# HansBambel/SmaAt-UNet

Hardware: NVIDIA H100
Metric: SmaAt-UNet fwd frames/sec @ B=32 12×288×288; depthwise % HBM roofline (higher is better)
Workload: dtype f32

## Files before the change

smaat_unet_b200/csrc/dsconv_fused.cu:

```cuda
#include <stdlib.h>

#include "tc_common.cuh"

namespace smaat {

struct DsParams {
  const float* dw_w;
  const float* dw_b;
  const float* scale;
  const float* shift;
  float* y;
  int64_t y_bstride;
  double* stats;
  const float* oc_w;
  const float* oc_b;
  float* oc_y;
  int C0, C1, H, W, Cout, relu, K;
  int tiles_x, tiles_y, npass, total_tiles, nchunks;
};

template <int N_TILE, int KPL, int PW, bool X3, bool A_SMEM>
struct DsCfg {
  static constexpr int PH = TC_BM / PW;
  static constexpr int BW = PW + 8, BH = PH + 2;
  static constexpr int CC = TC_BK / KPL;
  static constexpr int IN_BYTES = CC * BH * BW * 4;
  static constexpr int A_BYTES = TC_BM * TC_BK * 4;
  static constexpr int B_BYTES = N_TILE * TC_BK * 4;
  static constexpr int AST_BYTES = (X3 && A_SMEM ? 2 : 1) * A_BYTES;
  static constexpr int BST_BYTES = (X3 ? 2 : 1) * B_BYTES;
  static constexpr int OFF_ALO = A_BYTES;
  static constexpr int OFF_BLO = B_BYTES;
  static constexpr int NG = N_TILE > 64 ? 1 : 2;
  static constexpr int AS = X3 ? (A_SMEM ? (N_TILE > 64 ? 2 : 3) : 2 + NG) : 4;
  static constexpr int BS = X3 ? (A_SMEM && N_TILE > 64 ? 2 : 3) : 4;
  static constexpr int AFF_N = 512;
  static constexpr int BAR_BYTES = 512;
  static constexpr int IS_FIT = (224 * 1024 - 1024 - BAR_BYTES - 3 * AFF_N * 4 - AS * AST_BYTES - BS * BST_BYTES) / IN_BYTES;
  static constexpr int IS = IS_FIT > 8 ? 8 : IS_FIT;
  static constexpr int OFF_A = ((IS * IN_BYTES + 1023) / 1024) * 1024;
  static constexpr int OFF_BR = OFF_A + AS * AST_BYTES;
  static constexpr int OFF_BAR = OFF_BR + BS * BST_BYTES;
  static_assert((IS * NG + IS + 2 * AS + 2 * BS) * 8 <= BAR_BYTES, "barrier block");
  static constexpr int TOTAL = OFF_BAR + BAR_BYTES + 3 * AFF_N * 4 + 1024;
  static constexpr uint32_t B_TX = BST_BYTES;
  static constexpr int PROD_WARP = 12;
  static constexpr int THREADS = 384 + 128 * NG;
  static constexpr int REGS_LAUNCH = (65536 / THREADS) / 8 * 8;
  static constexpr int REGS_TMA = 24;
  static constexpr int REGS_PROD = N_TILE > 64 ? 104 : REGS_LAUNCH;
  static constexpr int REGS_MMA = ((THREADS / 128 * REGS_LAUNCH - REGS_TMA - NG * REGS_PROD) / 2) / 8 * 8;
  static constexpr int REGS_SUM = REGS_TMA + 2 * REGS_MMA + NG * REGS_PROD;
  static_assert(REGS_SUM <= THREADS / 128 * REGS_LAUNCH && REGS_MMA >= REGS_LAUNCH, "register budget");
  static constexpr int KS = (X3 && N_TILE == 64) ? 2 : TC_BK / 8;
  static_assert(IS >= 2, "input ring");
  static_assert(NG <= AS, "phase-parity barriers");
  static_assert(IN_BYTES % 128 == 0, "TMA destination alignment");
  static_assert(TOTAL <= 227 * 1024, "shared memory budget");
};

template <int N_TILE, int KPL, int PW, bool X3, bool A_SMEM>
__global__ void __launch_bounds__(DsCfg<N_TILE, KPL, PW, X3, A_SMEM>::THREADS, 1)
    dsconv_fused_kernel(const __grid_constant__ CUtensorMap map_in0, const __grid_constant__ CUtensorMap map_in1,
                        const __grid_constant__ CUtensorMap map_w, const __grid_constant__ CUtensorMap map_wlo,
                        const DsParams p) {
  using L = DsCfg<N_TILE, KPL, PW, X3, A_SMEM>;
  constexpr int PH = L::PH, BW = L::BW, BH = L::BH, CC = L::CC, IS = L::IS, AS = L::AS, BS = L::BS;
  extern __shared__ __align__(1024) unsigned char smem_dyn[];
  unsigned char* smem = smem_dyn + ((1024u - (smem_u32(smem_dyn) & 1023u)) & 1023u);
  unsigned char* a_base = smem + L::OFF_A;
  unsigned char* b_base = smem + L::OFF_BR;
  uint64_t* bars = reinterpret_cast<uint64_t*>(smem + L::OFF_BAR);
  uint64_t* in_full = bars;
  uint64_t* in_empty = in_full + IS * L::NG;
  uint64_t* a_full = in_empty + IS;
  uint64_t* a_empty = a_full + AS;
  uint64_t* b_full = a_empty + AS;
  uint64_t* b_empty = b_full + BS;
  float* aff = reinterpret_cast<float*>(smem + L::OFF_BAR + L::BAR_BYTES);

  const int warp = __shfl_sync(0xffffffffu, (int)(threadIdx.x >> 5), 0);
  const int lane = threadIdx.x & 31;
  const int nch = p.nchunks;
  const int tiles_per_img = p.tiles_x * p.tiles_y * p.npass;
  auto decode = [&](int tile, int& b, int& ty, int& tx, int& np) {
    b = tile / tiles_per_img;
    int t2 = tile - b * tiles_per_img;
    np = t2 % p.npass;
    t2 /= p.npass;
    ty = t2 / p.tiles_x;
    tx = t2 - ty * p.tiles_x;
  };

  if (warp == 0 && lane == 0) {
    tma_prefetch_desc(&map_in0);
    tma_prefetch_desc(&map_in1);
    tma_prefetch_desc(&map_w);
    if (X3) tma_prefetch_desc(&map_wlo);
    for (int s = 0; s < IS; ++s) {
      for (int g = 0; g < L::NG; ++g) mbar_init(&in_full[s * L::NG + g], 1);
      mbar_init(&in_empty[s], 128);
    }
    for (int s = 0; s < AS; ++s) {
      mbar_init(&a_full[s], 128);
      mbar_init(&a_empty[s], 8);
    }
    for (int s = 0; s < BS; ++s) {
      mbar_init(&b_full[s], 1);
      mbar_init(&b_empty[s], 8);
    }
    fence_barrier_init();
  }
  for (int c = threadIdx.x; c < L::AFF_N; c += blockDim.x) {
    aff[c] = (c < p.Cout && p.scale) ? __ldg(p.scale + c) : 1.f;
    aff[L::AFF_N + c] = (c < p.Cout && p.shift) ? __ldg(p.shift + c) : 0.f;
    aff[2 * L::AFF_N + c] = (c < p.Cout && p.oc_w) ? __ldg(p.oc_w + c) : 0.f;
  }
  __syncthreads();

  if (warp < 4) {
    regs_dealloc<L::REGS_TMA>();
    if (warp == 0 && lane == 0) {
      uint32_t gc = 0;
      for (int tile = blockIdx.x; tile < p.total_tiles; tile += gridDim.x) {
        int b, ty, tx, np;
        decode(tile, b, ty, tx, np);
        const int x0 = tx * PW, y0 = ty * PH;
        for (int i = 0; i < nch; ++i, ++gc) {
          const int s = gc % IS;
          mbar_wait(&in_empty[s], ((gc / IS) & 1u) ^ 1u);
          uint64_t* full = &in_full[s * L::NG + (int)(gc % (uint32_t)L::NG)];
          mbar_arrive_expect_tx(full, L::IN_BYTES);
          const int cb = i * CC;
          const CUtensorMap* m = (cb < p.C0) ? &map_in0 : &map_in1;
          const int cc = (cb < p.C0) ? cb : cb - p.C0;
          asm volatile(
              "cp.async.bulk.tensor.4d.shared::cluster.global.mbarrier::complete_tx::bytes [%0], [%1, {%3, %4, %5, %6}], [%2];" ::
                  "r"(smem_u32(smem + s * L::IN_BYTES)),
              "l"(reinterpret_cast<uint64_t>(m)), "r"(smem_u32(full)), "r"(x0 - 4), "r"(y0 - 1), "r"(cc), "r"(b)
              : "memory");
        }
      }
    }
    if (warp == 1 && lane == 0) {
      uint32_t gc = 0;
      for (int tile = blockIdx.x; tile < p.total_tiles; tile += gridDim.x) {
        int b, ty, tx, np;
        decode(tile, b, ty, tx, np);
        for (int i = 0; i < nch; ++i, ++gc) {
          const int sb = gc % BS;
          mbar_wait(&b_empty[sb], ((gc / BS) & 1u) ^ 1u);
          mbar_arrive_expect_tx(&b_full[sb], L::B_TX);
          tma_load_2d(b_base + sb * L::BST_BYTES, &map_w, &b_full[sb], i * TC_BK, np * N_TILE);
          if (X3) tma_load_2d(b_base + sb * L::BST_BYTES + L::OFF_BLO, &map_wlo, &b_full[sb], i * TC_BK, np * N_TILE);
        }
      }
    }
    return;
  }

  if (warp < L::PROD_WARP) {
    regs_alloc<L::REGS_MMA>();
    const int wg = (warp >> 2) - 1, wq = warp & 3;
    const int g = lane >> 2, t = lane & 3;
    const int m0 = A_SMEM ? 64 * wg + 16 * wq + g : tc_row_pixel(wg, wq, 0, g);
    const int m1 = A_SMEM ? m0 + 8 : tc_row_pixel(wg, wq, 1, g);
    const float act_lo = p.relu ? 0.f : -INFINITY;
    const int64_t P = (int64_t)p.H * p.W;
    uint32_t gc = 0;
    for (int tile = blockIdx.x; tile < p.total_tiles; tile += gridDim.x) {
      int b, ty, tx, np;
      decode(tile, b, ty, tx, np);
      float acc[N_TILE / 2];
#pragma unroll
      for (int i = 0; i < N_TILE / 2; ++i) acc[i] = 0.f;
      auto release = [&](uint32_t c) {
        __syncwarp();
        if (lane == 0) {
          mbar_arrive(&a_empty[c % AS]);
          mbar_arrive(&b_empty[c % BS]);
        }
      };
      auto wait_stages = [&](const unsigned char*& ast, uint64_t& bd, uint64_t& bl) {
        const int sa = gc % AS, sb = gc % BS;
        mbar_wait(&a_full[sa], (gc / AS) & 1u);
        mbar_wait(&b_full[sb], (gc / BS) & 1u);
        ast = a_base + sa * L::AST_BYTES;
        bd = make_kmajor_desc(smem_u32(b_base + sb * L::BST_BYTES));
        bl = make_kmajor_desc(smem_u32(b_base + sb * L::BST_BYTES + L::OFF_BLO));
      };
      if (A_SMEM) {
        for (int i = 0; i < nch; ++i, ++gc) {
          const unsigned char* ast;
          uint64_t bd0, bl0;
          wait_stages(ast, bd0, bl0);
          const uint32_t a_addr = smem_u32(ast) + (uint32_t)(wg * 64 * 128);
          const uint64_t ad0 = make_kmajor_desc(a_addr), al0 = make_kmajor_desc(a_addr + L::OFF_ALO);
          wgmma_fence();
#pragma unroll
          for (int kk = 0; kk < TC_BK / 8; ++kk) {
            Wgmma<N_TILE>::ss(acc, ad0 + (uint64_t)(2 * kk), bd0 + (uint64_t)(2 * kk), 1u);
            if (X3) {
              Wgmma<N_TILE>::ss(acc, al0 + (uint64_t)(2 * kk), bd0 + (uint64_t)(2 * kk), 1u);
              Wgmma<N_TILE>::ss(acc, ad0 + (uint64_t)(2 * kk), bl0 + (uint64_t)(2 * kk), 1u);
            }
          }
          wgmma_commit();
          wgmma_wait<1>();
          if (i > 0) release(gc - 1);
        }
        wgmma_wait0();
      } else {
        constexpr int KS = L::KS, GPC = (TC_BK / 8) / KS;
        const unsigned char* ast = nullptr;
        uint64_t bd0 = 0, bl0 = 0;
        auto group = [&](AFrags<X3, KS>& cur, AFrags<X3, KS>& prev, int q) {
          const int part = q % GPC;
          if (part == 0) wait_stages(ast, bd0, bl0);
          load_a_frags<X3, KS>(ast, part * KS, t, m0, m1, cur);
          mma_a_frags<N_TILE, X3, KS>(acc, cur, bd0, bl0, part * KS);
          wgmma_wait<1>();
          wgmma_keep(prev);
          if (part == 0 && q > 0) release(gc - 1);
          if (part == GPC - 1) ++gc;
        };
        AFrags<X3, KS> fa, fb;
        const int ngrp = nch * GPC;
        int q = 0;
        for (; q + 1 < ngrp; q += 2) {
          group(fa, fb, q);
          group(fb, fa, q + 1);
        }
        if (q < ngrp) group(fa, fb, q);
        wgmma_wait0();
        wgmma_keep(fa);
        wgmma_keep(fb);
      }
      wgmma_keep(acc);
      release(gc - 1);

      const int n0 = np * N_TILE;
      const int gy0 = ty * PH + m0 / PW, gx0 = tx * PW + m0 % PW;
      const int gy1 = ty * PH + m1 / PW, gx1 = tx * PW + m1 % PW;
      const bool v0 = gy0 < p.H && gx0 < p.W, v1 = gy1 < p.H && gx1 < p.W;
      const int64_t o0 = (int64_t)gy0 * p.W + gx0, o1 = (int64_t)gy1 * p.W + gx1;
      if (p.stats) {
        const double npix = (double)((__popc(__ballot_sync(0xffffffffu, v0)) + __popc(__ballot_sync(0xffffffffu, v1))) / 4);
#pragma unroll
        for (int j = 0; j < N_TILE / 8; ++j) {
#pragma unroll
          for (int e = 0; e < 2; ++e) {
            const float a = v0 ? acc[4 * j + e] : 0.f, bb = v1 ? acc[4 * j + 2 + e] : 0.f;
            const float s1 = frag_colsum(a + bb), s2 = frag_colsum(fmaf(a, a, bb * bb));
            const int c = 8 * j + 2 * t + e;
            if (lane < 4 && c < p.Cout) {
              const double sc = (double)aff[c], sh = (double)aff[L::AFF_N + c];
              atomicAdd(p.stats + c, sc * (double)s1 + npix * sh);
              atomicAdd(p.stats + p.Cout + c, sc * sc * (double)s2 + 2.0 * sc * sh * (double)s1 + npix * sh * sh);
            }
          }
        }
      }
      if (p.oc_y) {
        float d0 = 0.f, d1 = 0.f;
#pragma unroll
        for (int j = 0; j < N_TILE / 8; ++j) {
#pragma unroll
          for (int e = 0; e < 2; ++e) {
            const int c = 8 * j + 2 * t + e;
            const float sc = aff[c], sh = aff[L::AFF_N + c], w = aff[2 * L::AFF_N + c];
            d0 = fmaf(fmaxf(fmaf(acc[4 * j + e], sc, sh), act_lo), w, d0);
            d1 = fmaf(fmaxf(fmaf(acc[4 * j + 2 + e], sc, sh), act_lo), w, d1);
          }
        }
        d0 += __shfl_xor_sync(0xffffffffu, d0, 1);
        d0 += __shfl_xor_sync(0xffffffffu, d0, 2);
        d1 += __shfl_xor_sync(0xffffffffu, d1, 1);
        d1 += __shfl_xor_sync(0xffffffffu, d1, 2);
        const float ob = p.oc_b ? __ldg(p.oc_b) : 0.f;
        if (t == 0) {
          if (v0) p.oc_y[(int64_t)b * P + o0] = d0 + ob;
          if (v1) p.oc_y[(int64_t)b * P + o1] = d1 + ob;
        }
      } else {
        float* yb = p.y + (int64_t)b * p.y_bstride;
#pragma unroll
        for (int j = 0; j < N_TILE / 8; ++j) {
#pragma unroll
          for (int e = 0; e < 2; ++e) {
            const int c = n0 + 8 * j + 2 * t + e;
            if (c < p.Cout) {
              const float sc = aff[c], sh = aff[L::AFF_N + c];
              float* yc = yb + (int64_t)c * P;
              if (v0) yc[o0] = fmaxf(fmaf(acc[4 * j + e], sc, sh), act_lo);
              if (v1) yc[o1] = fmaxf(fmaf(acc[4 * j + 2 + e], sc, sh), act_lo);
            }
          }
        }
      }
    }
    return;
  }

  {
    if (L::REGS_PROD < L::REGS_LAUNCH) regs_dealloc<L::REGS_PROD>();
    const int g = (warp - L::PROD_WARP) >> 2;
    const int t = threadIdx.x - 32 * L::PROD_WARP - 128 * g;
    const int Cin = p.C0 + p.C1;
    uint32_t gc = 0, iph = 0;
    for (int tile = blockIdx.x; tile < p.total_tiles; tile += gridDim.x) {
      for (int i = 0; i < nch; ++i, ++gc) {
        if ((int)(gc % (uint32_t)L::NG) != g) continue;
        const int s = gc % IS;
        float wr[KPL][9], br[KPL];
        auto task_channel = [&](int task) { return (PW == 32) ? (task >> 3) : (((task >> 4) << 1) | ((task >> 2) & 1)); };
        auto load_weights = [&](int task) {
          const int gch = i * CC + task_channel(task);
          const bool chv = gch < Cin;
#pragma unroll
          for (int kk = 0; kk < KPL; ++kk) {
            const int gk = gch * KPL + kk;
#pragma unroll
            for (int w9 = 0; w9 < 9; ++w9) wr[kk][w9] = chv ? __ldg(p.dw_w + (int64_t)gk * 9 + w9) : 0.f;
            br[kk] = (chv && p.dw_b) ? __ldg(p.dw_b + gk) : 0.f;
          }
        };
        load_weights(t);
        mbar_wait(&in_full[s * L::NG + g], (iph >> s) & 1u);
        iph ^= 1u << s;
        const int sa = gc % AS;
        mbar_wait(&a_empty[sa], ((gc / AS) & 1u) ^ 1u);
        unsigned char* my_op = a_base + sa * L::AST_BYTES;
        const float* in_stage = reinterpret_cast<const float*>(smem + s * L::IN_BYTES);
#pragma unroll 1
        for (int task = t; task < CC * 8; task += 128) {
          int ci, qc, rg;
          if (PW == 32) {
            ci = task >> 3; qc = task & 7; rg = 0;
          } else {
            qc = task & 3; ci = ((task >> 4) << 1) | ((task >> 2) & 1); rg = (task >> 3) & 1;
          }
          constexpr int NQ = PW / 4;
          const int c0 = qc << 2, r0 = rg << 2;
          if (task != t) load_weights(task);
          const float* trow = in_stage + (ci * BH + r0) * BW + c0 + 3;
          float win[3][6];
          const bool lb = (qc == 0), rb = (qc == NQ - 1);
          const int edge = lb ? 0 : 5;
          auto load_row = [&](float* wl, int r) {
            const float4 a = *reinterpret_cast<const float4*>(trow + r * BW + 1);
            float left = __shfl_up_sync(0xffffffffu, a.w, 1), right = __shfl_down_sync(0xffffffffu, a.x, 1);
            if (lb | rb) {
              const float e = trow[r * BW + edge];
              if (lb) left = e; else right = e;
            }
            wl[0] = left; wl[1] = a.x; wl[2] = a.y; wl[3] = a.z; wl[4] = a.w; wl[5] = right;
          };
#pragma unroll
          for (int r = 0; r < 2; ++r) load_row(win[r], r);
#pragma unroll
          for (int rr = 0; rr < 4; ++rr) {
            load_row(win[(rr + 2) % 3], rr + 2);
            const float* w0 = win[rr % 3];
            const float* w1 = win[(rr + 1) % 3];
            const float* w2 = win[(rr + 2) % 3];
            const int m = (r0 + rr) * PW + c0;
#pragma unroll
            for (int kk = 0; kk < KPL; ++kk) {
              float o4[4];
#pragma unroll
              for (int j = 0; j < 4; ++j) {
                float a = br[kk];
                a = fmaf(wr[kk][0], w0[j], a); a = fmaf(wr[kk][1], w0[j + 1], a); a = fmaf(wr[kk][2], w0[j + 2], a);
                a = fmaf(wr[kk][3], w1[j], a); a = fmaf(wr[kk][4], w1[j + 1], a); a = fmaf(wr[kk][5], w1[j + 2], a);
                a = fmaf(wr[kk][6], w2[j], a); a = fmaf(wr[kk][7], w2[j + 1], a); a = fmaf(wr[kk][8], w2[j + 2], a);
                o4[j] = a;
              }
              if (A_SMEM) {
                const int kr = ci * KPL + kk;
#pragma unroll
                for (int j = 0; j < 4; ++j) {
                  const uint32_t off = kmajor_offset(m + j, kr);
                  const float h = X3 ? tf32_hi(o4[j]) : o4[j];
                  *reinterpret_cast<float*>(my_op + off) = h;
                  if (X3) *reinterpret_cast<float*>(my_op + L::OFF_ALO + off) = o4[j] - h;
                }
                continue;
              }
              *reinterpret_cast<float4*>(my_op + a_tile_offset(ci * KPL + kk, m)) = make_float4(o4[0], o4[1], o4[2], o4[3]);
            }
          }
        }
        if (A_SMEM) fence_proxy_async_smem();
        mbar_arrive(&a_full[sa]);
        mbar_arrive(&in_empty[s]);
      }
    }
  }
}

template <int N_TILE, int KPL, int PW, bool X3, bool A_SMEM>
static int launch_ds(const CUtensorMap& m0, const CUtensorMap& m1, const CUtensorMap& mw, const CUtensorMap& mwl, DsParams p,
                     int B, cudaStream_t st) {
  using L = DsCfg<N_TILE, KPL, PW, X3, A_SMEM>;
  auto kern = dsconv_fused_kernel<N_TILE, KPL, PW, X3, A_SMEM>;
  static std::atomic<uint64_t> attr_mask{0};
  if (first_use_on_device(attr_mask)) {
    cudaError_t e = cudaFuncSetAttribute(kern, cudaFuncAttributeMaxDynamicSharedMemorySize, L::TOTAL);
    if (e != cudaSuccess) return fail(SMAAT_E_CUDA, "dsconv: smem attribute (%d B): %s", L::TOTAL, cudaGetErrorString(e));
    int r = check_reg_budget((const void*)kern, L::THREADS, L::REGS_SUM, "dsconv");
    if (r) return r;
  }
  p.tiles_x = ceil_div(p.W, PW);
  p.tiles_y = ceil_div(p.H, L::PH);
  p.npass = ceil_div(p.Cout, N_TILE);
  const int64_t total = (int64_t)B * p.tiles_x * p.tiles_y * p.npass;
  SMAAT_REQUIRE(total < (1ll << 31), "dsconv: too many tiles");
  p.total_tiles = (int)total;
  p.nchunks = ceil_div(p.C0 + p.C1, L::CC);
  const int grid = p.total_tiles < num_sms() ? p.total_tiles : num_sms();
  kern<<<grid, L::THREADS, L::TOTAL, st>>>(m0, m1, mw, mwl, p);
  SMAAT_LAUNCH_CHECK("smaat_dsconv_fwd");
  return SMAAT_OK;
}

static int pick_pw(int H, int W) {
  double best = 1e9;
  int pw = 0;
  const int cand[2] = {32, 16};
  for (int i = 0; i < 2; ++i) {
    const int c = cand[i], ph = TC_BM / c;
    const double waste = ((double)ceil_div(W, c) * c / W) * ((double)ceil_div(H, ph) * ph / H);
    if (waste < best - 1e-9) {
      best = waste;
      pw = c;
    }
  }
  return best <= 1.35 ? pw : 0;
}

static bool ds_eligible(const float* x0, int C0, int64_t bs0, const float* x1, int C1, int64_t bs1, const float* pw_w,
                        const float* pw_w_lo, int H, int W, int k, int Cout, bool stats, bool outconv) {
  if (k != 1 && k != 2) return false;
  if (Cout < 8 || Cout > 512 || (Cout > 128 && (Cout % 128 != 0 || stats || outconv))) return false;
  if (W % 4 != 0 || !aligned16(x0) || bs0 % 4 != 0) return false;
  if (C1 > 0 && (!aligned16(x1) || bs1 % 4 != 0 || C0 % (TC_BK / k) != 0)) return false;
  const int K = k * (C0 + C1);
  if (K % 4 != 0 || !aligned16(pw_w) || (pw_w_lo && !aligned16(pw_w_lo))) return false;
  return pick_pw(H, W) != 0;
}

static std::atomic<int> g_ds_impl{-1};
static int ds_impl() {
  int v = g_ds_impl.load(std::memory_order_relaxed);
  if (v < 0) {
    const char* e = getenv("SMAAT_DS_IMPL");
    v = e ? atoi(e) : 0;
    if (v < 0 || v > 2) v = 0;
    g_ds_impl.store(v, std::memory_order_relaxed);
  }
  return v;
}

}

using namespace smaat;

extern "C" int smaat_set_dsconv_impl(int impl) {
  SMAAT_REQUIRE(impl >= 0 && impl <= 2, "set_dsconv_impl: 0 = auto, 1 = A operand from shared memory, 2 = A operand from registers");
  g_ds_impl.store(impl, std::memory_order_relaxed);
  return SMAAT_OK;
}

extern "C" int smaat_dsconv_eligible2(const float* x0, int C0, int64_t x0_bstride, const float* x1, int C1, int64_t x1_bstride,
                                      const float* pw_w, int H, int W, int k, int Cout, int with_stats) {
  return ds_eligible(x0, C0, x0_bstride, x1, C1, x1_bstride, pw_w, nullptr, H, W, k, Cout, with_stats != 0, false) ? 1 : 0;
}

extern "C" int smaat_dsconv_eligible(const float* x0, int C0, int64_t x0_bstride, const float* x1, int C1, int64_t x1_bstride,
                                     const float* pw_w, int H, int W, int k, int Cout) {
  return smaat_dsconv_eligible2(x0, C0, x0_bstride, x1, C1, x1_bstride, pw_w, H, W, k, Cout, 0);
}

static int dsconv_run(const float* x0, int C0, int64_t x0_bstride, const float* x1, int C1, int64_t x1_bstride, const float* dw_w,
                      const float* dw_b, const float* pw_w, const float* pw_w_lo, const float* scale, const float* shift, float* y,
                      int64_t y_bstride, double* stats, const float* oc_w, const float* oc_b, float* oc_y, int B, int H, int W,
                      int k, int Cout, int relu, int mode, void* stream) {
  SMAAT_REQUIRE(x0 && dw_w && pw_w && (y || oc_y), "dsconv: null pointer");
  SMAAT_REQUIRE(B > 0 && C0 > 0 && C1 >= 0 && H > 0 && W > 0 && Cout > 0, "dsconv: bad shape");
  SMAAT_REQUIRE(C1 == 0 || x1, "dsconv: C1=%d but x1 is null", C1);
  SMAAT_REQUIRE(mode == SMAAT_PW_TF32 || mode == SMAAT_PW_TF32X3, "dsconv: mode must be SMAAT_PW_TF32 or SMAAT_PW_TF32X3");
  SMAAT_REQUIRE(mode != SMAAT_PW_TF32X3 || pw_w_lo, "dsconv: TF32X3 needs pw_w_lo (see smaat_split_tf32)");
  SMAAT_REQUIRE(oc_y || y_bstride >= (int64_t)Cout * H * W, "dsconv: y batch stride too small");
  SMAAT_REQUIRE(!oc_y || (oc_w && !stats), "dsconv+outconv: needs the OutConv weight and no batch statistics");
  if (!ds_eligible(x0, C0, x0_bstride, x1, C1, x1_bstride, pw_w, pw_w_lo, H, W, k, Cout, stats != nullptr, oc_y != nullptr))
    return fail(SMAAT_E_UNSUPPORTED, "dsconv: shape not taken by the fused kernel (k=%d Cout=%d H=%d W=%d); use dw3x3 + pw1x1", k,
                Cout, H, W);
  cudaStream_t st = (cudaStream_t)stream;
  const int pw = pick_pw(H, W);
  const int ph = TC_BM / pw;
  const int n_tile = Cout > 64 ? 128 : 64;
  const int cc = TC_BK / k;
  const bool x3 = mode == SMAAT_PW_TF32X3;
  const bool a_smem = ds_impl() == 1;
  const int K = k * (C0 + C1);

  CUtensorMap m0, m1, mw, mwl;
  const uint32_t box[4] = {(uint32_t)(pw + 8), (uint32_t)(ph + 2), (uint32_t)cc, 1u};
  {
    const uint64_t dims[4] = {(uint64_t)W, (uint64_t)H, (uint64_t)C0, (uint64_t)B};
    const uint64_t str[4] = {0, (uint64_t)W * 4, (uint64_t)H * W * 4, (uint64_t)x0_bstride * 4};
    int r = make_tmap_f32(&m0, x0, 4, dims, str, box, CU_TENSOR_MAP_SWIZZLE_NONE, "dsconv(x0)");
    if (r) return r;
    m1 = m0;
  }
  if (C1 > 0) {
    const uint64_t dims[4] = {(uint64_t)W, (uint64_t)H, (uint64_t)C1, (uint64_t)B};
    const uint64_t str[4] = {0, (uint64_t)W * 4, (uint64_t)H * W * 4, (uint64_t)x1_bstride * 4};
    int r = make_tmap_f32(&m1, x1, 4, dims, str, box, CU_TENSOR_MAP_SWIZZLE_NONE, "dsconv(x1)");
    if (r) return r;
  }
  {
    const uint64_t dims[2] = {(uint64_t)K, (uint64_t)Cout};
    const uint64_t str[2] = {0, (uint64_t)K * 4};
    const uint32_t wbox[2] = {(uint32_t)TC_BK, (uint32_t)n_tile};
    int r = make_tmap_f32(&mw, pw_w, 2, dims, str, wbox, CU_TENSOR_MAP_SWIZZLE_128B, "dsconv(w)");
    if (r) return r;
    mwl = mw;
    if (x3) {
      r = make_tmap_f32(&mwl, pw_w_lo, 2, dims, str, wbox, CU_TENSOR_MAP_SWIZZLE_128B, "dsconv(w_lo)");
      if (r) return r;
    }
  }
  DsParams p;
  p.dw_w = dw_w; p.dw_b = dw_b; p.scale = scale; p.shift = shift; p.y = y; p.y_bstride = y_bstride; p.stats = stats;
  p.oc_w = oc_w; p.oc_b = oc_b; p.oc_y = oc_y;
  p.C0 = C0; p.C1 = C1; p.H = H; p.W = W; p.Cout = Cout; p.relu = relu; p.K = K;
  p.tiles_x = p.tiles_y = p.npass = p.total_tiles = p.nchunks = 0;

#define DS_DISPATCH(NT, KP, PWv)                                                                           \
  return x3 ? (a_smem ? launch_ds<NT, KP, PWv, true, true>(m0, m1, mw, mwl, p, B, st)                       \
                      : launch_ds<NT, KP, PWv, true, false>(m0, m1, mw, mwl, p, B, st))                     \
            : (a_smem ? launch_ds<NT, KP, PWv, false, true>(m0, m1, mw, mwl, p, B, st)                      \
                      : launch_ds<NT, KP, PWv, false, false>(m0, m1, mw, mwl, p, B, st))
  if (n_tile == 64) {
    if (k == 2) { if (pw == 32) { DS_DISPATCH(64, 2, 32); } else { DS_DISPATCH(64, 2, 16); } }
    else        { if (pw == 32) { DS_DISPATCH(64, 1, 32); } else { DS_DISPATCH(64, 1, 16); } }
  } else {
    if (k == 2) { if (pw == 32) { DS_DISPATCH(128, 2, 32); } else { DS_DISPATCH(128, 2, 16); } }
    else        { if (pw == 32) { DS_DISPATCH(128, 1, 32); } else { DS_DISPATCH(128, 1, 16); } }
  }
#undef DS_DISPATCH
}

extern "C" int smaat_dsconv_fwd(const float* x0, int C0, int64_t x0_bstride, const float* x1, int C1, int64_t x1_bstride,
                                const float* dw_w, const float* dw_b, const float* pw_w, const float* pw_w_lo,
                                const float* scale, const float* shift, float* y, int64_t y_bstride, double* stats, int B, int H,
                                int W, int k, int Cout, int relu, int mode, void* stream) {
  SMAAT_REQUIRE(y, "dsconv: null output");
  return dsconv_run(x0, C0, x0_bstride, x1, C1, x1_bstride, dw_w, dw_b, pw_w, pw_w_lo, scale, shift, y, y_bstride, stats, nullptr,
                    nullptr, nullptr, B, H, W, k, Cout, relu, mode, stream);
}

extern "C" int smaat_dsconv_outconv_fwd(const float* x0, int C0, int64_t x0_bstride, const float* x1, int C1, int64_t x1_bstride,
                                        const float* dw_w, const float* dw_b, const float* pw_w, const float* pw_w_lo,
                                        const float* scale, const float* shift, const float* oc_w, const float* oc_b,
                                        float* logits, int B, int H, int W, int k, int Cout, int relu, int mode, void* stream) {
  SMAAT_REQUIRE(oc_w && logits, "dsconv+outconv: null pointer");
  return dsconv_run(x0, C0, x0_bstride, x1, C1, x1_bstride, dw_w, dw_b, pw_w, pw_w_lo, scale, shift, nullptr, 0, nullptr, oc_w, oc_b,
                    logits, B, H, W, k, Cout, relu, mode, stream);
}
```

Measured before the change: 2480.

## Stage dsconv output in swizzled shared memory and write with TMA bulk stores

Replaces per-thread global stores of the fused depthwise-pointwise output with a per-warpgroup staging path. Accumulators are transposed within quads, the affine and activation are applied, and results go into double-buffered swizzled shared tiles that a leader thread writes out with 4D TMA stores. The aim is fully coalesced output writes and store traffic that overlaps the next tile's MMA. The staging buffers take shared memory from the input ring, which may reduce pipeline depth. Each store also adds named-barrier syncs and shuffles.

```diff
diff --git a/smaat_unet_b200/csrc/dsconv_fused.cu b/smaat_unet_b200/csrc/dsconv_fused.cu
--- a/smaat_unet_b200/csrc/dsconv_fused.cu
+++ b/smaat_unet_b200/csrc/dsconv_fused.cu
@@ -36,11 +36,20 @@
   static constexpr int BS = X3 ? (A_SMEM && N_TILE > 64 ? 2 : 3) : 4;
   static constexpr int AFF_N = 512;
   static constexpr int BAR_BYTES = 512;
-  static constexpr int IS_FIT = (224 * 1024 - 1024 - BAR_BYTES - 3 * AFF_N * 4 - AS * AST_BYTES - BS * BST_BYTES) / IN_BYTES;
+  static constexpr int FREE = 224 * 1024 - 1024 - BAR_BYTES - 3 * AFF_N * 4 - AS * AST_BYTES - BS * BST_BYTES;
+  static constexpr int ST_BOX = 32 * 64 * 4;
+  static constexpr int ST_WANT = 2;
+  static constexpr int ST_BUFS = (FREE - 2 * ST_WANT * ST_BOX) / IN_BYTES >= 2 ? ST_WANT
+                                 : (FREE - 2 * ST_BOX) / IN_BYTES >= 2     ? 1
+                                                                           : 0;
+  static constexpr int ST_BYTES = 2 * ST_BUFS * ST_BOX;
+  static_assert(ST_BUFS > 0 || (FREE - 2 * ST_BOX) / IN_BYTES < 2, "staging falls back only where one buffer does not fit");
+  static constexpr int IS_FIT = (FREE - ST_BYTES) / IN_BYTES;
   static constexpr int IS = IS_FIT > 8 ? 8 : IS_FIT;
   static constexpr int OFF_A = ((IS * IN_BYTES + 1023) / 1024) * 1024;
   static constexpr int OFF_BR = OFF_A + AS * AST_BYTES;
-  static constexpr int OFF_BAR = OFF_BR + BS * BST_BYTES;
+  static constexpr int OFF_ST = OFF_BR + BS * BST_BYTES;
+  static constexpr int OFF_BAR = OFF_ST + ST_BYTES;
   static_assert((IS * NG + IS + 2 * AS + 2 * BS) * 8 <= BAR_BYTES, "barrier block");
   static constexpr int TOTAL = OFF_BAR + BAR_BYTES + 3 * AFF_N * 4 + 1024;
   static constexpr uint32_t B_TX = BST_BYTES;
@@ -59,11 +68,37 @@
   static_assert(TOTAL <= 227 * 1024, "shared memory budget");
 };
 
+__device__ __forceinline__ void tma_store_4d(const CUtensorMap* m, uint32_t src, int c0, int c1, int c2, int c3) {
+  asm volatile("cp.async.bulk.tensor.4d.global.shared::cta.bulk_group [%0, {%2, %3, %4, %5}], [%1];" ::"l"(
+                   reinterpret_cast<uint64_t>(m)),
+               "r"(src), "r"(c0), "r"(c1), "r"(c2), "r"(c3)
+               : "memory");
+}
+__device__ __forceinline__ void bulk_commit() { asm volatile("cp.async.bulk.commit_group;" ::: "memory"); }
+template <int N>
+__device__ __forceinline__ void bulk_wait_read() { asm volatile("cp.async.bulk.wait_group.read %0;" ::"n"(N) : "memory"); }
+__device__ __forceinline__ void bulk_wait_all() { asm volatile("cp.async.bulk.wait_group 0;" ::: "memory"); }
+__device__ __forceinline__ void wg_sync(int id) { asm volatile("bar.sync %0, 128;" ::"r"(id) : "memory"); }
+
+__device__ __forceinline__ void quad_transpose(float (&v)[4], int q) {
+  const bool h1 = q & 2, h0 = q & 1;
+#pragma unroll
+  for (int e = 0; e < 2; ++e) {
+    const float r = __shfl_xor_sync(0xffffffffu, h1 ? v[e] : v[e + 2], 8);
+    if (h1) v[e] = r; else v[e + 2] = r;
+  }
+#pragma unroll
+  for (int e = 0; e < 4; e += 2) {
+    const float r = __shfl_xor_sync(0xffffffffu, h0 ? v[e] : v[e + 1], 4);
+    if (h0) v[e] = r; else v[e + 1] = r;
+  }
+}
+
 template <int N_TILE, int KPL, int PW, bool X3, bool A_SMEM>
 __global__ void __launch_bounds__(DsCfg<N_TILE, KPL, PW, X3, A_SMEM>::THREADS, 1)
     dsconv_fused_kernel(const __grid_constant__ CUtensorMap map_in0, const __grid_constant__ CUtensorMap map_in1,
                         const __grid_constant__ CUtensorMap map_w, const __grid_constant__ CUtensorMap map_wlo,
-                        const DsParams p) {
+                        const __grid_constant__ CUtensorMap map_y, const DsParams p) {
   using L = DsCfg<N_TILE, KPL, PW, X3, A_SMEM>;
   constexpr int PH = L::PH, BW = L::BW, BH = L::BH, CC = L::CC, IS = L::IS, AS = L::AS, BS = L::BS;
   extern __shared__ __align__(1024) unsigned char smem_dyn[];
@@ -97,6 +132,7 @@
     tma_prefetch_desc(&map_in1);
     tma_prefetch_desc(&map_w);
     if (X3) tma_prefetch_desc(&map_wlo);
+    if (L::ST_BUFS && !p.oc_y) tma_prefetch_desc(&map_y);
     for (int s = 0; s < IS; ++s) {
       for (int g = 0; g < L::NG; ++g) mbar_init(&in_full[s * L::NG + g], 1);
       mbar_init(&in_empty[s], 128);
@@ -167,6 +203,15 @@
     const int m1 = A_SMEM ? m0 + 8 : tc_row_pixel(wg, wq, 1, g);
     const float act_lo = p.relu ? 0.f : -INFINITY;
     const int64_t P = (int64_t)p.H * p.W;
+    constexpr int SW_MASK = PW == 32 ? 7 : 3;
+    const int quad = g & 3, slot = quad ^ (t & 2);
+    const int st_ch = 2 * t + (slot & 1);
+    const int st_px = ((slot & 2) ? m1 : m0) - quad - 64 * wg;
+    const uint32_t st_a0 = (uint32_t)(st_ch * 256 + st_px * 4);
+    const uint32_t st_off = st_a0 ^ (((st_a0 >> 7) & SW_MASK) << 4);
+    const uint32_t st_base = smem_u32(smem + L::OFF_ST) + (uint32_t)(wg * L::ST_BUFS * L::ST_BOX);
+    const bool st_leader = (threadIdx.x & 127) == 0;
+    uint32_t st_n = 0;
     uint32_t gc = 0;
     for (int tile = blockIdx.x; tile < p.total_tiles; tile += gridDim.x) {
       int b, ty, tx, np;
@@ -282,6 +327,37 @@
           if (v0) p.oc_y[(int64_t)b * P + o0] = d0 + ob;
           if (v1) p.oc_y[(int64_t)b * P + o1] = d1 + ob;
         }
+      } else if (L::ST_BUFS) {
+        const int y_half = ty * PH + wg * (PH / 2);
+#pragma unroll
+        for (int s = 0; s < N_TILE / 32; ++s) {
+          if (n0 + 32 * s >= p.Cout) break;
+          const uint32_t buf = st_base + (st_n % L::ST_BUFS) * L::ST_BOX;
+          if (st_leader) bulk_wait_read<L::ST_BUFS - 1>();
+          wg_sync(2 + wg);
+#pragma unroll
+          for (int jj = 0; jj < 4; ++jj) {
+            const int j = 4 * s + jj;
+            float v[4];
+#pragma unroll
+            for (int q = 0; q < 4; ++q) v[q] = (t & 2) ? acc[4 * j + (q ^ 2)] : acc[4 * j + q];
+            quad_transpose(v, quad);
+            const int c = n0 + 8 * j + st_ch;
+            const float sc = aff[c], sh = aff[L::AFF_N + c];
+            const float4 o = make_float4(fmaxf(fmaf(v[0], sc, sh), act_lo), fmaxf(fmaf(v[1], sc, sh), act_lo),
+                                         fmaxf(fmaf(v[2], sc, sh), act_lo), fmaxf(fmaf(v[3], sc, sh), act_lo));
+            asm volatile("st.shared.v4.f32 [%0], {%1, %2, %3, %4};" ::"r"(buf + st_off + 2048u * jj), "f"(o.x), "f"(o.y),
+                         "f"(o.z), "f"(o.w)
+                         : "memory");
+          }
+          fence_proxy_async_smem();
+          wg_sync(2 + wg);
+          if (st_leader) {
+            tma_store_4d(&map_y, buf, tx * PW, y_half, n0 + 32 * s, b);
+            bulk_commit();
+          }
+          ++st_n;
+        }
       } else {
         float* yb = p.y + (int64_t)b * p.y_bstride;
 #pragma unroll
@@ -299,6 +375,7 @@
         }
       }
     }
+    if (L::ST_BUFS && st_leader) bulk_wait_all();
     return;
   }
 
@@ -400,8 +477,8 @@
 }
 
 template <int N_TILE, int KPL, int PW, bool X3, bool A_SMEM>
-static int launch_ds(const CUtensorMap& m0, const CUtensorMap& m1, const CUtensorMap& mw, const CUtensorMap& mwl, DsParams p,
-                     int B, cudaStream_t st) {
+static int launch_ds(const CUtensorMap& m0, const CUtensorMap& m1, const CUtensorMap& mw, const CUtensorMap& mwl,
+                     const CUtensorMap& my, DsParams p, int B, cudaStream_t st) {
   using L = DsCfg<N_TILE, KPL, PW, X3, A_SMEM>;
   auto kern = dsconv_fused_kernel<N_TILE, KPL, PW, X3, A_SMEM>;
   static std::atomic<uint64_t> attr_mask{0};
@@ -419,7 +496,7 @@
   p.total_tiles = (int)total;
   p.nchunks = ceil_div(p.C0 + p.C1, L::CC);
   const int grid = p.total_tiles < num_sms() ? p.total_tiles : num_sms();
-  kern<<<grid, L::THREADS, L::TOTAL, st>>>(m0, m1, mw, mwl, p);
+  kern<<<grid, L::THREADS, L::TOTAL, st>>>(m0, m1, mw, mwl, my, p);
   SMAAT_LAUNCH_CHECK("smaat_dsconv_fwd");
   return SMAAT_OK;
 }
@@ -440,8 +517,10 @@
 }
 
 static bool ds_eligible(const float* x0, int C0, int64_t bs0, const float* x1, int C1, int64_t bs1, const float* pw_w,
-                        const float* pw_w_lo, int H, int W, int k, int Cout, bool stats, bool outconv) {
+                        const float* pw_w_lo, const float* y, int64_t y_bstride, int H, int W, int k, int Cout, bool stats,
+                        bool outconv) {
   if (k != 1 && k != 2) return false;
+  if (y && (!aligned16(y) || y_bstride % 4 != 0)) return false;
   if (Cout < 8 || Cout > 512 || (Cout > 128 && (Cout % 128 != 0 || stats || outconv))) return false;
   if (W % 4 != 0 || !aligned16(x0) || bs0 % 4 != 0) return false;
   if (C1 > 0 && (!aligned16(x1) || bs1 % 4 != 0 || C0 % (TC_BK / k) != 0)) return false;
@@ -474,7 +553,8 @@
 
 extern "C" int smaat_dsconv_eligible2(const float* x0, int C0, int64_t x0_bstride, const float* x1, int C1, int64_t x1_bstride,
                                       const float* pw_w, int H, int W, int k, int Cout, int with_stats) {
-  return ds_eligible(x0, C0, x0_bstride, x1, C1, x1_bstride, pw_w, nullptr, H, W, k, Cout, with_stats != 0, false) ? 1 : 0;
+  return ds_eligible(x0, C0, x0_bstride, x1, C1, x1_bstride, pw_w, nullptr, nullptr, 0, H, W, k, Cout, with_stats != 0, false) ? 1
+                                                                                                                                : 0;
 }
 
 extern "C" int smaat_dsconv_eligible(const float* x0, int C0, int64_t x0_bstride, const float* x1, int C1, int64_t x1_bstride,
@@ -493,9 +573,12 @@
   SMAAT_REQUIRE(mode != SMAAT_PW_TF32X3 || pw_w_lo, "dsconv: TF32X3 needs pw_w_lo (see smaat_split_tf32)");
   SMAAT_REQUIRE(oc_y || y_bstride >= (int64_t)Cout * H * W, "dsconv: y batch stride too small");
   SMAAT_REQUIRE(!oc_y || (oc_w && !stats), "dsconv+outconv: needs the OutConv weight and no batch statistics");
-  if (!ds_eligible(x0, C0, x0_bstride, x1, C1, x1_bstride, pw_w, pw_w_lo, H, W, k, Cout, stats != nullptr, oc_y != nullptr))
-    return fail(SMAAT_E_UNSUPPORTED, "dsconv: shape not taken by the fused kernel (k=%d Cout=%d H=%d W=%d); use dw3x3 + pw1x1", k,
-                Cout, H, W);
+  if (!ds_eligible(x0, C0, x0_bstride, x1, C1, x1_bstride, pw_w, pw_w_lo, oc_y ? nullptr : y, y_bstride, H, W, k, Cout,
+                   stats != nullptr, oc_y != nullptr))
+    return fail(SMAAT_E_UNSUPPORTED,
+                "dsconv: shape or output layout not taken by the fused kernel (k=%d Cout=%d H=%d W=%d, y 16-byte aligned with a "
+                "batch stride that is a multiple of 4); use dw3x3 + pw1x1",
+                k, Cout, H, W);
   cudaStream_t st = (cudaStream_t)stream;
   const int pw = pick_pw(H, W);
   const int ph = TC_BM / pw;
@@ -532,6 +615,14 @@
       if (r) return r;
     }
   }
+  CUtensorMap my = m0;
+  if (!oc_y) {
+    const uint64_t dims[4] = {(uint64_t)W, (uint64_t)H, (uint64_t)Cout, (uint64_t)B};
+    const uint64_t str[4] = {0, (uint64_t)W * 4, (uint64_t)H * W * 4, (uint64_t)y_bstride * 4};
+    const uint32_t ybox[4] = {(uint32_t)pw, (uint32_t)(ph / 2), 32u, 1u};
+    int r = make_tmap_f32(&my, y, 4, dims, str, ybox, pw == 32 ? CU_TENSOR_MAP_SWIZZLE_128B : CU_TENSOR_MAP_SWIZZLE_64B, "dsconv(y)");
+    if (r) return r;
+  }
   DsParams p;
   p.dw_w = dw_w; p.dw_b = dw_b; p.scale = scale; p.shift = shift; p.y = y; p.y_bstride = y_bstride; p.stats = stats;
   p.oc_w = oc_w; p.oc_b = oc_b; p.oc_y = oc_y;
@@ -539,10 +630,10 @@
   p.tiles_x = p.tiles_y = p.npass = p.total_tiles = p.nchunks = 0;
 
 #define DS_DISPATCH(NT, KP, PWv)                                                                           \
-  return x3 ? (a_smem ? launch_ds<NT, KP, PWv, true, true>(m0, m1, mw, mwl, p, B, st)                       \
-                      : launch_ds<NT, KP, PWv, true, false>(m0, m1, mw, mwl, p, B, st))                     \
-            : (a_smem ? launch_ds<NT, KP, PWv, false, true>(m0, m1, mw, mwl, p, B, st)                      \
-                      : launch_ds<NT, KP, PWv, false, false>(m0, m1, mw, mwl, p, B, st))
+  return x3 ? (a_smem ? launch_ds<NT, KP, PWv, true, true>(m0, m1, mw, mwl, my, p, B, st)                   \
+                      : launch_ds<NT, KP, PWv, true, false>(m0, m1, mw, mwl, my, p, B, st))                 \
+            : (a_smem ? launch_ds<NT, KP, PWv, false, true>(m0, m1, mw, mwl, my, p, B, st)                  \
+                      : launch_ds<NT, KP, PWv, false, false>(m0, m1, mw, mwl, my, p, B, st))
   if (n_tile == 64) {
     if (k == 2) { if (pw == 32) { DS_DISPATCH(64, 2, 32); } else { DS_DISPATCH(64, 2, 16); } }
     else        { if (pw == 32) { DS_DISPATCH(64, 1, 32); } else { DS_DISPATCH(64, 1, 16); } }
```

New measurement: 2628 (median of 6 runs). 1.06x the previous value.
